# YimingQiao/Chunk-Compaction-in-Vectorized-Execution-SIMD

Measured on AMD Instinct MI355X. Metric: probe tuples/sec + achieved HBM GB/s, 1B-row int64 join at 1/2/4/8 GPUs, higher is better.
Workload: dtype int64; 1 GPU; C2: 1xMI355X linear-probe, 64M build / 1B probe int64 uniform keys, chunk=2048; table=linear_probing, layout=device, n_build=67108864, n_probe_per_gpu=1073741824, chunk=2048, parallelism=dp1

## Files before the change

chunk-compaction-in-vectorized-execution-simd_amd/ccj.py:

```python
from __future__ import annotations

import ctypes as C
import os
import subprocess

HERE = os.path.dirname(os.path.abspath(__file__))
LIB_PATH = os.environ.get("CCJ_LIB_PATH") or os.path.join(HERE, "libccj.so")

LP, CHAIN = 0, 1
LAYOUT_REFERENCE, LAYOUT_DEVICE = 0, 1
FLAG_CAP_OVERFLOW, FLAG_ROUND_OVERFLOW, FLAG_BAD_INPUT, FLAG_PART_OVERFLOW = 1, 2, 4, 8
PART_EXACT = 1
PART_ROWS = 2
PART_RANK = 4
PART_SHARE = 8

_lib = None
ABI_VERSION = 15


class CCJError(RuntimeError):
    pass


class TableInfo(C.Structure):
    _fields_ = [("kind", C.c_int32), ("layout", C.c_int32), ("n_keys", C.c_uint64), ("size", C.c_uint64),
                ("max_dup", C.c_uint64), ("max_rounds", C.c_uint32), ("reserved", C.c_uint32),
                ("d_table", C.c_void_p), ("d_bucket_off", C.c_void_p)]


class TableArrays(C.Structure):
    _fields_ = [("d_table", C.c_void_p), ("positions", C.c_uint64), ("d_row", C.c_void_p),
                ("d_bucket_off", C.c_void_p), ("d_bucket16", C.c_void_p), ("d_bucket8", C.c_void_p),
                ("n_bucket8", C.c_uint64), ("d_bucket_filter", C.c_void_p), ("n_filter_words", C.c_uint64)]


class ProbeArgs(C.Structure):
    _fields_ = [("keys", C.c_void_p), ("sel", C.c_void_p), ("counts", C.c_void_p), ("n_rows", C.c_uint64),
                ("chunk", C.c_uint32), ("max_rounds", C.c_uint32), ("cap", C.c_uint64),
                ("out_count", C.c_void_p), ("out_sel", C.c_void_p), ("out_payload", C.c_void_p),
                ("out_rounds", C.c_void_p), ("out_round_counts", C.c_void_p), ("status", C.c_void_p),
                ("out_pos", C.c_void_p), ("n_payload_cols", C.c_uint32), ("reserved2", C.c_uint32),
                ("out_payload_cols", C.c_void_p * 8)]


class CompactArgs(C.Structure):
    _fields_ = [("count", C.c_void_p), ("sel", C.c_void_p), ("payload", C.c_void_p), ("rounds", C.c_void_p),
                ("round_counts", C.c_void_p), ("n_chunks", C.c_uint64), ("cap", C.c_uint64),
                ("max_rounds", C.c_uint32), ("chunk", C.c_uint32), ("n_cols", C.c_uint32), ("threshold", C.c_uint32),
                ("cols", C.c_void_p * 16), ("out_cols", C.c_void_p * 16), ("out_payload", C.c_void_p),
                ("out_row", C.c_void_p), ("out_chunk_counts", C.c_void_p), ("out_cap_rows", C.c_uint64),
                ("out_n_chunks", C.c_void_p), ("workspace", C.c_void_p), ("workspace_bytes", C.c_size_t),
                ("status", C.c_void_p), ("key_cols", C.c_uint32)]


EXPORTS = ["ccj_last_error", "ccj_abi_version", "ccj_device_init", "ccj_table_build_reference",
           "ccj_table_build_from_host", "ccj_table_build_on_device", "ccj_table_get_info", "ccj_table_free",
           "ccj_probe", "ccj_gen_uniform_keys", "ccj_probe_cost", "ccj_result_checksum",
           "ccj_compact_workspace_size", "ccj_compact", "ccj_partition_workspace_size", "ccj_partition_by_owner",
           "ccj_result_checksum_mapped", "ccj_gen_reference_keys", "ccj_table_set_payload",
           "ccj_table_build_rank_index",
           "ccj_probe_partitioned_workspace_size", "ccj_probe_partitioned", "ccj_probe_partitioned_positions",
           "ccj_pipeline_create",
           "ccj_pipeline_run", "ccj_pipeline_free", "ccj_pipeline_checksum", "ccj_partition_by_owner_fixed",
           "ccj_segment_chunk_counts", "ccj_pipeline_set_thresholds", "ccj_gen_c3_keys",
           "ccj_partition_grouped_workspace_size", "ccj_partition_by_owner_grouped", "ccj_partition_grouped_sub_cap",
           "ccj_probe_ordered_workspace_size", "ccj_probe_ordered", "ccj_probe_visits",
           "ccj_stream_create_cu_masked", "ccj_stream_destroy", "ccj_device_cus", "ccj_copy_device",
           "ccj_table_get_arrays", "ccj_probe_cost_walk", "ccj_set_phase_events", "ccj_build_hash",
           "ccj_last_gather_kernel"]

MAX_JOINS = 8
COMPACT_NONE, COMPACT_FULL = 0, 1


class PipelineResult(C.Structure):
    _fields_ = [("n_out", C.c_uint64), ("cols", C.c_void_p * MAX_JOINS), ("payload", C.c_void_p * MAX_JOINS),
                ("chunks_in", C.c_uint64 * MAX_JOINS), ("rows_in", C.c_uint64 * MAX_JOINS),
                ("rows_out", C.c_uint64 * MAX_JOINS), ("level_ms", C.c_float * MAX_JOINS)]


def build(force: bool = False) -> str:
    if force or not os.path.exists(LIB_PATH):
        subprocess.run(["make", "-C", HERE, "-j8"], check=True)
    return LIB_PATH


def lib():
    global _lib
    if _lib is None:
        if not os.path.exists(LIB_PATH):
            raise CCJError(f"{LIB_PATH} missing: run `make -C {HERE}` (or __graft_entry__.build())")
        L = C.CDLL(LIB_PATH)
        vp, u64, i32 = C.c_void_p, C.c_uint64, C.c_int
        L.ccj_last_error.restype = C.c_char_p
        L.ccj_abi_version.restype = i32
        if L.ccj_abi_version() != ABI_VERSION:
            raise CCJError(f"{LIB_PATH} has ABI {L.ccj_abi_version()}, this binding needs {ABI_VERSION}: "
                           f"rebuild it (`make -C {HERE}`)")
        L.ccj_build_hash.restype = C.c_char_p
        L.ccj_last_gather_kernel.restype = C.c_char_p
        L.ccj_device_init.argtypes = [i32]
        L.ccj_table_build_reference.argtypes = [i32, u64, u64, i32, vp, C.POINTER(vp)]
        L.ccj_table_build_from_host.argtypes = [i32, vp, u64, C.POINTER(vp)]
        L.ccj_table_build_on_device.argtypes = [i32, vp, u64, vp, C.POINTER(vp)]
        L.ccj_table_get_info.argtypes = [vp, C.POINTER(TableInfo)]
        L.ccj_table_get_arrays.argtypes = [vp, C.POINTER(TableArrays)]
        L.ccj_table_free.argtypes = [vp]
        L.ccj_table_set_payload.argtypes = [vp, vp, C.c_uint32, vp]
        L.ccj_table_build_rank_index.argtypes = [vp, vp]
        L.ccj_probe_partitioned_workspace_size.restype = C.c_size_t
        L.ccj_probe_partitioned_workspace_size.argtypes = [vp, u64, C.c_uint32]
        L.ccj_probe_partitioned_positions.restype = u64
        L.ccj_probe_partitioned_positions.argtypes = [vp, u64, C.c_uint32]
        L.ccj_probe_partitioned.argtypes = [vp, C.POINTER(ProbeArgs), C.c_uint32, vp, vp, C.c_size_t, vp]
        L.ccj_probe.argtypes = [vp, C.POINTER(ProbeArgs), vp]
        L.ccj_probe_ordered_workspace_size.restype = C.c_size_t
        L.ccj_probe_ordered_workspace_size.argtypes = [vp, u64, C.c_uint32]
        L.ccj_probe_ordered.argtypes = [vp, C.POINTER(ProbeArgs), vp, C.c_size_t, vp]
        L.ccj_gen_uniform_keys.argtypes = [vp, u64, u64, u64, u64, vp]
        L.ccj_gen_reference_keys.argtypes = [vp, u64, u64, u64, u64, vp]
        L.ccj_gen_c3_keys.argtypes = [vp, u64, u64, u64, u64, u64, C.c_uint32, vp]
        L.ccj_probe_cost.argtypes = [vp, vp, u64, vp, vp]
        L.ccj_probe_cost_walk.argtypes = [vp, vp, u64, vp, vp]
        L.ccj_set_phase_events.argtypes = [C.POINTER(vp), C.c_uint32]
        L.ccj_probe_visits.argtypes = [vp, vp, vp, C.c_uint32, C.c_uint32, vp, vp, vp]
        L.ccj_compact_workspace_size.restype = C.c_size_t
        L.ccj_compact_workspace_size.argtypes = [u64, u64, C.c_uint32, C.c_uint32, C.c_uint32]
        L.ccj_compact.argtypes = [C.POINTER(CompactArgs), vp]
        L.ccj_partition_workspace_size.restype = C.c_size_t
        L.ccj_partition_workspace_size.argtypes = [u64, C.c_uint32]
# ... 135 lines not shown
        out = torch.empty(n, dtype=torch.int64, device=torch.device("cuda", torch.cuda.current_device()))
    check(lib().ccj_gen_c3_keys(_ptr(out), n, seed, first_row, n_build, cf, hit_ppm, _stream(stream)),
          "ccj_gen_c3_keys")
    return out


def gen_reference_keys(first: int, n: int, n_total: int, cf: int = 1, out=None, stream=None):
    import torch
    if out is None:
        out = torch.empty(n, dtype=torch.int64, device=torch.device("cuda", torch.cuda.current_device()))
    check(lib().ccj_gen_reference_keys(_ptr(out), first, n, n_total, cf, _stream(stream)), "ccj_gen_reference_keys")
    return out


class Table:
    def __init__(self, handle: C.c_void_p):
        self._h = handle
        info = TableInfo()
        check(lib().ccj_table_get_info(handle, C.byref(info)), "ccj_table_get_info")
        self.kind, self.layout = info.kind, info.layout
        self.n_keys, self.size = info.n_keys, info.size
        self.max_dup, self.max_rounds = info.max_dup, info.max_rounds
        self.d_table, self.d_bucket_off = info.d_table, info.d_bucket_off

    @classmethod
    def reference(cls, kind: int, n: int, cf: int = 1, layout: int = LAYOUT_REFERENCE, stream=None):
        h = C.c_void_p()
        check(lib().ccj_table_build_reference(kind, n, cf, layout, _stream(stream), C.byref(h)),
              "ccj_table_build_reference")
        return cls(h)

    @classmethod
    def from_host(cls, kind: int, keys):
        import numpy as np
        keys = np.ascontiguousarray(keys, dtype=np.int64)
        h = C.c_void_p()
        check(lib().ccj_table_build_from_host(kind, keys.ctypes.data_as(C.c_void_p), len(keys), C.byref(h)),
              "ccj_table_build_from_host")
        return cls(h)

    @classmethod
    def on_device(cls, kind: int, d_keys, stream=None):
        h = C.c_void_p()
        check(lib().ccj_table_build_on_device(kind, _ptr(d_keys), d_keys.numel(), _stream(stream), C.byref(h)),
              "ccj_table_build_on_device")
        return cls(h)

    def free(self):
        if self._h:
            lib().ccj_table_free(self._h)
            self._h = None

    def __del__(self):
        try:
            self.free()
        except Exception:
            pass

    def arrays(self):
        import numpy as np
        import torch
        a = TableArrays()
        check(lib().ccj_table_get_arrays(self._h, C.byref(a)), "ccj_table_get_arrays")
        torch.cuda.synchronize()

        def get(ptr, n, dt):
            return _d2h_bytes(ptr, n * np.dtype(dt).itemsize).view(dt)

        out = dict(table=get(a.d_table, a.positions, np.int64), row=get(a.d_row, a.positions, np.uint32))
# ... 414 lines not shown
```

chunk-compaction-in-vectorized-execution-simd_amd/csrc/ccj_api.hip:

```cpp
#include <algorithm>
#include <cstdlib>
#include <cstdio>
#include <cstring>
#include <map>
#include <memory>
#include <mutex>
#include <new>
#include <string>
#include <unordered_map>
#include <vector>

#include "ccj_internal.h"
#include "ccj_tuning.h"

namespace {

thread_local std::string g_err;

thread_local hipEvent_t g_phase[4] = {};
thread_local uint32_t g_n_phase = 0;
thread_local uint32_t g_phase_next = 0;
void phase_mark(hipStream_t s, uint32_t i) {
  if (i < g_n_phase && g_phase[i]) (void)hipEventRecord(g_phase[i], s);
  if (i + 1 > g_phase_next) g_phase_next = i + 1;
// ... 130 lines not shown
  if (e == hipSuccess) e = hipMalloc((void **)&t->d_ckeys, nck * 8);
  if (e == hipSuccess) e = ccj::launch_fill(t->d_ckeys, nck, -1, s);
  if (e == hipSuccess) e = ccj::launch_rank_index(t->d_table, size, t->d_occ, t->d_pre, cnt, s);
  if (e == hipSuccess) e = ccj::launch_rank_compact_keys(t->d_table, size, t->d_occ, t->d_pre, t->d_ckeys, s);
  if (e == hipSuccess) e = hipStreamSynchronize(s);
  if (cnt) (void)hipFree(cnt);
  if (e != hipSuccess) {
    for (void *q : {(void *)t->d_occ, (void *)t->d_pre, (void *)t->d_ckeys})
      if (q) (void)hipFree(q);
    t->d_occ = nullptr;
    t->d_pre = nullptr;
    t->d_ckeys = nullptr;
    return hip_fail(e, "LP window index");
  }
  t->rank_wbits = pl.window_bits;
  return CCJ_OK;
}
#else
int build_rank_index(ccj_table *, hipStream_t) {
  return fail(CCJ_ERR_INVALID, "ccj_table_build_rank_index: the rank walk is built into libccj_tuning.so only");
}
#endif

int build_lp_host(const int64_t *keys, uint64_t n, ccj_table **out) {
  const uint64_t size = lp_num_slots(n);
  if (size > (1ull << 32)) return fail(CCJ_ERR_LIMIT, "LP table larger than 2^32 slots");
  std::vector<int64_t> slots(size, -1);
  std::vector<uint32_t> rows(size < 4 ? 4 : size, ccj::kNoRow);
  const uint64_t mask = size - 1;
  for (uint64_t i = 0; i < n; ++i) {
    uint64_t s = ccj::murmurhash64((uint64_t)keys[i]) & mask;
    while (slots[s] != -1) s = (s + 1) & mask;
    slots[s] = keys[i];
    if (keys[i] != -1) rows[s] = (uint32_t)i;
  }
  std::unique_ptr<ccj_table> t(new ccj_table());
  t->info.kind = CCJ_TABLE_LP;
  t->info.layout = CCJ_LAYOUT_REFERENCE;
  t->info.n_keys = n;
  t->info.size = size;
  lp_host_stats(slots, &t->info.max_rounds, &t->info.max_dup);
  if (slots.size() < 4) slots.resize(4, -1);
  void *d = nullptr;
  int rc = upload(&d, slots.data(), slots.size() * sizeof(int64_t), "LP slots");
  if (rc) return rc;
  t->d_table = (int64_t *)d;
  t->positions = slots.size();
  rc = upload(&d, rows.data(), rows.size() * sizeof(uint32_t), "LP slot rows");
  if (rc) {
    (void)hipFree(t->d_table);
    return rc;
  }
  t->d_row = (uint32_t *)d;
  t->info.d_table = t->d_table;
  (void)hipGetDevice(&t->device);
  *out = t.release();
  return CCJ_OK;
}

int build_chain_host(const int64_t *keys, uint64_t n, ccj_table **out) {
  if (n >= (1ull << 32)) return fail(CCJ_ERR_LIMIT, "chaining table needs < 2^32 keys (uint32 CSR)");
  const uint64_t size = chain_num_buckets(n);
  const uint64_t mask = size - 1;
  std::vector<uint32_t> off(size + 1, 0);
  std::vector<uint32_t> bucket(n);
  for (uint64_t i = 0; i < n; ++i) {
    bucket[i] = (uint32_t)(ccj::murmurhash64((uint64_t)keys[i]) & mask);
    off[bucket[i] + 1]++;
  }
  uint32_t longest = 0;
  for (uint64_t b = 0; b < size; ++b) {
    longest = std::max(longest, off[b + 1]);
    off[b + 1] += off[b];
  }
  std::vector<int64_t> chain(n);
  std::vector<uint32_t> rows;
  {
    std::vector<uint32_t> fill(off.begin(), off.end() - 1);
// ... 134 lines not shown
  if (n_seg) best = std::max<uint64_t>(best, carry + st[0]);
  t->info.kind = CCJ_TABLE_LP;
  t->info.layout = CCJ_LAYOUT_DEVICE;
  t->info.n_keys = n;
  t->info.size = size;
  t->info.max_rounds = (uint32_t)best;
  uint64_t dup = known_dup;
  if (!dup && n) {
    uint32_t *d_dup = nullptr, h_dup = 0;
    e = hipMalloc(&d_dup, sizeof(uint32_t));
    if (e == hipSuccess) e = ccj::launch_lp_max_dup(t->d_table, size, (uint32_t)std::min<uint64_t>(best, size), d_dup, s);
    if (e == hipSuccess) e = hipMemcpyAsync(&h_dup, d_dup, sizeof(uint32_t), hipMemcpyDeviceToHost, s);
    if (e == hipSuccess) e = hipStreamSynchronize(s);
    if (d_dup) (void)hipFree(d_dup);
    if (e != hipSuccess) {
      cleanup();
      return hip_fail(e, "device LP build (max dup)");
    }
    dup = h_dup;
  }
  t->info.max_dup = dup ? dup : 1;
  t->info.d_table = t->d_table;
  (void)hipGetDevice(&t->device);
  *out = t.release();
  return CCJ_OK;
}

void zipf_table(uint64_t n, uint32_t *t) {
  double hn = 0.0;
  for (uint64_t r = 1; r <= n; ++r) hn += 1.0 / (double)r;
  uint32_t j = 0;
  double h = 0.0;
  for (uint64_t r = 1; r <= n && j < ccj::kZipfBuckets; ++r) {
    h += 1.0 / (double)r;
    while (j < ccj::kZipfBuckets && h * (double)ccj::kZipfBuckets > (double)j * hn) t[j++] = (uint32_t)r;
  }
  while (j < ccj::kZipfBuckets) t[j++] = (uint32_t)(n ? n : 1);
  t[ccj::kZipfBuckets] = (uint32_t)(n + 1);
}

}

extern "C" {

const char *ccj_last_error(void) { return g_err.c_str(); }

// ... 94 lines not shown
    return fail(CCJ_ERR_INVALID, "ccj_table_set_payload: bad argument");
  if (!t->d_row) return fail(CCJ_ERR_INVALID, "ccj_table_set_payload: table has no row map");
  void *d = nullptr;
  if (hipMalloc(&d, t->positions * n_cols * sizeof(int64_t)) != hipSuccess)
    return fail(CCJ_ERR_OOM, "payload: hipMalloc failed");
  hipError_t e = ccj::launch_scatter_payload(d_payload, n_cols, t->d_row, t->positions, (int64_t *)d,
                                             (hipStream_t)stream);
  if (e == hipSuccess) e = hipStreamSynchronize((hipStream_t)stream);
  if (e != hipSuccess) {
    (void)hipFree(d);
    return hip_fail(e, "payload scatter");
  }
  if (t->d_pay) (void)hipFree(t->d_pay);
  t->d_pay = (int64_t *)d;
  t->n_pay = n_cols;
  return CCJ_OK;
}

int ccj_table_build_rank_index(ccj_table *t, ccj_stream stream) {
  if (!t) return fail(CCJ_ERR_INVALID, "ccj_table_build_rank_index: null table");
  return build_rank_index(t, (hipStream_t)stream);
}

int ccj_table_free(ccj_table *t) {
  if (!t) return CCJ_OK;
  if (t->d_table) (void)hipFree(t->d_table);
  if (t->d_off) (void)hipFree(t->d_off);
  if (t->d_bucket) (void)hipFree(t->d_bucket);
  if (t->d_bucket8) (void)hipFree(t->d_bucket8);
  if (t->d_filt) (void)hipFree(t->d_filt);
  if (t->d_row) (void)hipFree(t->d_row);
  if (t->d_pay) (void)hipFree(t->d_pay);
  if (t->d_occ) (void)hipFree(t->d_occ);
  if (t->d_pre) (void)hipFree(t->d_pre);
  if (t->d_ckeys) (void)hipFree(t->d_ckeys);
  delete t;
  return CCJ_OK;
}

namespace {
int fill_probe_params(const ccj_table *t, const ccj_probe_args *a, ccj::ProbeParams &p) {
  if (!t || !a) return fail(CCJ_ERR_INVALID, "ccj_probe: null table/args");
  if (a->chunk == 0 || a->chunk > ccj::kMaxChunk) return fail(CCJ_ERR_INVALID, "ccj_probe: chunk must be 1..2048");
  if (a->out_round_counts && a->max_rounds == 0) return fail(CCJ_ERR_INVALID, "ccj_probe: max_rounds == 0");
  if (a->n_rows && (!a->out_count || !a->out_sel || !a->keys))
    return fail(CCJ_ERR_INVALID, "ccj_probe: missing buffer");
  p = ccj::ProbeParams{};
  p.table = t->d_table;
// ... 79 lines not shown
  const size_t rank = 0;
  (void)t;
#endif
  return align256(L.positions * 8) + align256(fixed > exact ? fixed : exact) + rank;
}
size_t part_ws_sub_bytes(const ccj_table *t, const PartLayout &L, uint32_t chunk) {
  if (!t->n_pay || !L.pl.lo_bits) return 0;
  const uint64_t out_chunks = (L.positions + chunk - 1) / chunk;
  return align256(out_chunks * 8 * 4);
}
}

size_t ccj_probe_partitioned_workspace_size(const ccj_table *t, uint64_t n_rows, uint32_t chunk) {
  if (!t) return 0;
  const PartLayout L = part_layout(t, n_rows, chunk);
  return part_ws_base_bytes(t, L, n_rows) + part_ws_sub_bytes(t, L, chunk);
}

int ccj_probe_partitioned(const ccj_table *t, const ccj_probe_args *a, uint32_t flags, uint32_t *out_row_map,
                          void *ws, size_t ws_bytes, ccj_stream stream) {
  PhaseScope phase_scope((hipStream_t)stream);
  ccj::ProbeParams p;
  if (int rc = fill_probe_params(t, a, p)) return rc;
  if (t->info.kind == CCJ_TABLE_CHAIN && (a->out_pos || a->n_payload_cols))
    return fail(CCJ_ERR_INVALID, "ccj_probe_partitioned: positions / payload columns need an LP table");
  if (a->sel) return fail(CCJ_ERR_INVALID, "ccj_probe_partitioned: sel must be NULL");
  if (a->counts && (flags & CCJ_PART_EXACT))
    return fail(CCJ_ERR_INVALID, "ccj_probe_partitioned: input chunk counts need the one-pass split (no CCJ_PART_EXACT)");
  if (a->out_round_counts)
    return fail(CCJ_ERR_INVALID, "ccj_probe_partitioned: no round counts (no Next boundaries in partition order)");
  if ((a->out_pos || a->n_payload_cols) && t->info.size < 16)
    return fail(CCJ_ERR_INVALID, "ccj_probe_partitioned: positions / payload columns need a table of >= 16 slots");
  if (a->n_rows >= (1ull << 32)) return fail(CCJ_ERR_LIMIT, "ccj_probe_partitioned: n_rows must be < 2^32");
  if (flags & ~(CCJ_PART_EXACT | CCJ_PART_ROWS | CCJ_PART_RANK | CCJ_PART_SHARE))
    return fail(CCJ_ERR_INVALID, "ccj_probe_partitioned: unknown flags");
#ifdef CCJ_RANK_WALK
  if ((flags & CCJ_PART_RANK) && !t->d_ckeys && rank_index_applies(t))
    return fail(CCJ_ERR_INVALID, "ccj_probe_partitioned: CCJ_PART_RANK needs ccj_table_build_rank_index first");
#else
  if (flags & CCJ_PART_RANK)
    return fail(CCJ_ERR_INVALID, "ccj_probe_partitioned: CCJ_PART_RANK: the rank walk is built into libccj_tuning.so only");
#endif
  const bool rows = (flags & CCJ_PART_ROWS) != 0;
  if (rows && (!a->out_payload || p.cap != a->chunk || t->info.max_dup > 1 || t->info.kind != CCJ_TABLE_LP ||
               t->info.size < 16 || ((a->out_pos || a->n_payload_cols) && t->info.size > (1ull << 31))))
    return fail(CCJ_ERR_INVALID, "ccj_probe_partitioned: CCJ_PART_ROWS needs an LP table of >= 16 slots with distinct "
// ... 516 lines not shown
```

chunk-compaction-in-vectorized-execution-simd_amd/csrc/ccj_internal.h:

```cpp
#pragma once

#include <hip/hip_runtime.h>

#include <cstdint>
#include <string>

#include "ccj.h"

struct ccj_table {
  ccj_table_info info;
  int64_t *d_table = nullptr;
  uint32_t *d_off = nullptr;
  int64_t *d_bucket = nullptr;
  uint64_t *d_bucket8 = nullptr;
  uint32_t *d_filt = nullptr;
  uint32_t *d_row = nullptr;
  uint64_t positions = 0;
  int64_t *d_pay = nullptr;
  uint32_t n_pay = 0;
  int device = 0;
  uint64_t *d_occ = nullptr;
  uint32_t *d_pre = nullptr;
  int64_t *d_ckeys = nullptr;
  uint32_t rank_wbits = 0;
};

namespace ccj {

__host__ __device__ __forceinline__ uint64_t murmurhash64(uint64_t x) {
  x ^= x >> 32;
  x *= 0xd6e8feb86659fd93ULL;
  x ^= x >> 32;
  x *= 0xd6e8feb86659fd93ULL;
  x ^= x >> 32;
  return x;
}

__host__ __device__ __forceinline__ uint32_t murmurhash64_hi(uint64_t x) {
  constexpr uint64_t kC = 0xd6e8feb86659fd93ULL;
  x ^= x >> 32;
  x *= kC;
  x ^= x >> 32;
  const uint32_t lo = (uint32_t)x, hi = (uint32_t)(x >> 32);
  return (uint32_t)(((uint64_t)lo * (uint32_t)kC) >> 32) + lo * (uint32_t)(kC >> 32) + hi * (uint32_t)kC;
}

__host__ __device__ __forceinline__ uint32_t bucket_fp(uint64_t h) { return (uint32_t)(h >> 52); }
__host__ __device__ __forceinline__ uint32_t rec8_first(uint64_t r, uint32_t kfp) {
  const uint32_t st = (uint32_t)r, len = (uint32_t)(r >> 32) & 0xFFu;
  const bool m0 = ((uint32_t)(r >> 40) & 0xFFFu) == kfp;
  const bool m1 = len >= 2u && ((uint32_t)(r >> 52) & 0xFFFu) == kfp;
  const uint32_t c = m0 ? st : m1 ? st + 1u : st + 2u;
  return c < st + len ? c : st + len;
}

constexpr int kWave = 64;
constexpr int kWavesPerBlock = 4;
constexpr uint32_t kMaxChunk = 2048;
constexpr uint32_t kMaxParts = 64;

struct ProbeParams {
  const int64_t *table;
  const uint32_t *off;
  const longlong2 *bucket;
  const uint64_t *bucket8;
  uint32_t mask;
  const int64_t *keys;
  const uint32_t *sel;
  const uint32_t *counts;
  uint64_t n_rows;
  uint64_t n_chunks;
  uint32_t chunk;
  uint32_t max_rounds;
  uint64_t cap;
  uint32_t *out_count;
  uint32_t *out_sel;
  int64_t *out_payload;
  uint32_t *out_rounds;
  uint32_t *out_round_counts;
  uint32_t *status;
  uint32_t *out_pos;
  const int64_t *pay;
  uint32_t n_pay;
  uint32_t pay_stride;
  int64_t *out_cols[CCJ_MAX_PAYLOAD_COLS];
// ... 30 lines not shown

hipError_t launch_probe(int kind, const ProbeParams &p, hipStream_t s);
hipError_t launch_probe_flat(int kind, const ProbeParams &p, hipStream_t s);
hipError_t launch_ordered_walk(int kind, const ProbeParams &p, hipStream_t s);
uint32_t stream_cus(hipStream_t s);
hipError_t launch_unsplit_words(const uint2 *runs, const uint32_t *ovf_runs, const uint16_t *row_loc,
                                const void *w_pos, void *w_row, uint64_t n, uint32_t parts, uint32_t tile,
                                uint32_t *status, hipStream_t s, bool w16);
hipError_t launch_ordered_emit(int kind, const ProbeParams &p, hipStream_t s);
hipError_t launch_gather_payload(const ProbeParams &p, const uint32_t *pos, hipStream_t s, uint32_t parts = 0,
                                 uint64_t cpp = 0);
const char *last_gather_kernel();
hipError_t launch_gen_reference_keys(int64_t *out, uint64_t first, uint64_t n, uint64_t n_total, uint64_t cf,
                                     hipStream_t s);
hipError_t launch_fill(int64_t *p, uint64_t n, int64_t v, hipStream_t s);
hipError_t launch_iota_u32(uint32_t *p, uint64_t n, hipStream_t s);
hipError_t launch_copy16(const void *src, void *dst, uint64_t n16, hipStream_t s);
hipError_t launch_lp_insert(const int64_t *keys, uint64_t n, int64_t *slots, uint32_t *slot_row, uint32_t mask,
                            hipStream_t s);
hipError_t launch_scatter_payload(const int64_t *src, uint32_t n_cols, const uint32_t *row, uint64_t positions,
                                  int64_t *dst, hipStream_t s);
hipError_t launch_lp_max_dup(const int64_t *slots, uint64_t n_slots, uint32_t max_run, uint32_t *out, hipStream_t s);
hipError_t launch_lp_runs(const int64_t *slots, uint64_t n_slots, uint32_t *seg_stats, hipStream_t s);
int build_chain_device(const int64_t *d_keys, uint64_t n, hipStream_t s, uint64_t known_dup, ccj_table **out);
hipError_t build_chain_filter(ccj_table *t, hipStream_t s);
constexpr uint64_t kRunSegment = 4096;
hipError_t launch_gen_c3(int64_t *out, uint64_t n, uint64_t seed, uint64_t first_row, uint64_t n_build, uint64_t cf,
                         uint32_t hit_ppm, const uint32_t *zipf, hipStream_t s);
constexpr uint32_t kZipfBits = 16, kZipfBuckets = 1u << kZipfBits;
hipError_t launch_gen_uniform(int64_t *out, uint64_t n, uint64_t seed, uint64_t first_row, uint64_t range,
                              hipStream_t s);
hipError_t launch_probe_visits(int kind, const int64_t *table, const uint32_t *off, uint32_t mask,
                               const int64_t *keys, const uint32_t *sel, uint32_t count, uint32_t max_rounds,
                               int64_t *vals, uint32_t *len, hipStream_t s);
hipError_t launch_probe_cost(int kind, const int64_t *table, const uint32_t *off, uint32_t mask,
                             const int64_t *keys, uint64_t n, unsigned long long *acc, hipStream_t s,
                             bool walk = false);
hipError_t launch_result_checksum(const uint32_t *count, const uint32_t *sel, const int64_t *payload,
                                  uint64_t n_chunks, uint64_t cap, uint32_t chunk, uint64_t row_base,
                                  const uint64_t *row_map, unsigned long long *acc, hipStream_t s);

int api_fail(int code, const std::string &msg);
int api_check_device();

size_t compact_workspace(uint64_t n_chunks, uint64_t cap, uint32_t chunk, uint32_t max_rounds, uint32_t threshold);
hipError_t launch_compact(const ccj_compact_args &a, hipStream_t s);
// ... 72 lines not shown
```

chunk-compaction-in-vectorized-execution-simd_amd/csrc/ccj_kernels.hip:

```cpp
#include <cstdlib>
#include <string>

#include "ccj_internal.h"
#include "ccj_tuning.h"

namespace ccj {
namespace {

__device__ __forceinline__ uint32_t lane_prefix(uint64_t m) {
  return __builtin_amdgcn_mbcnt_hi((uint32_t)(m >> 32), __builtin_amdgcn_mbcnt_lo((uint32_t)m, 0u));
}

template <int KIND>
__device__ __forceinline__ void emit_extra(const ProbeParams &p, uint64_t obase, uint64_t o, int64_t k, uint32_t r) {
  if (!p.out_pos && p.n_pay == 0) return;
  const uint32_t h = (uint32_t)murmurhash64((uint64_t)k) & p.mask;
  const uint32_t pos = KIND == CCJ_TABLE_LP ? ((h + r) & p.mask) : p.off[h] + r;
  if (p.out_pos) p.out_pos[obase + o] = pos;
  if (p.n_pay) {
    const int64_t *row = p.pay + (uint64_t)pos * p.pay_stride;
    for (uint32_t c = 0; c < p.n_pay; ++c) p.out_cols[c][obase + o] = row[c];
  }
}

// ... 2428 lines not shown
      walk_finish(p, sm, c, lane, lane_rounds, 0u, t0, t1, t2, steps);
      return;
    }
  }
  const uint32_t overflow = walk_emit<kWaveRows>(p, sm, c, w0, wend, lane);
  walk_finish(p, sm, c, lane, lane_rounds, overflow, t0, t1, t2, steps);
}

#ifdef CCJ_TUNING
template <int AUX, int KJ>
__device__ __forceinline__ void stage_keys_aux(const int64_t *keys, uint32_t phys, uint32_t w0, uint32_t wend,
                                               uint32_t lane, int64_t (&k)[KJ]) {
  const auto rs = __builtin_amdgcn_make_buffer_rsrc(const_cast<int64_t *>(keys), (short)0, (int)(phys * 8), 0x00020000);
#pragma unroll
  for (int j = 0; j < KJ; ++j) {
    const uint32_t i = w0 + (uint32_t)(j >> 1) * 128u + 2u * lane + (uint32_t)(j & 1);
    k[j] = (int64_t)__builtin_amdgcn_raw_buffer_load_b64(rs, (int)(i * 8), 0, AUX);
  }
#pragma unroll
  for (int j = 0; j < KJ; ++j)
    if (w0 + (uint32_t)(j >> 1) * 128u + 2u * lane + (uint32_t)(j & 1) >= wend) k[j] = 0;
}
#endif
template <bool POS, int NB = 1>
__global__ __launch_bounds__(kWave * 4, POS && NB == 1 ? 5 : 1) void probe_walk2(ProbeParams p) {
  constexpr int NW = 4;
  constexpr uint32_t kWaveRows = kMaxChunk / NW;
  constexpr int kJ = (int)(kWaveRows / kWave);
  __shared__ Walk1Shared<NB, NW> sm;
  const uint32_t tid = threadIdx.x, lane = tid & (kWave - 1), wave = tid / kWave;
  unsigned long long t0, t1, t2;
  uint32_t steps = 0;
  CCJ_STAMP(t0);
  const uint64_t c = walk_chunk_index(p);
  const uint64_t base = c * p.chunk;
  const uint32_t phys = flat_phys(p, base);
  const uint32_t w0 = wave * kWaveRows;
  const uint32_t wend = phys > w0 ? (phys - w0 < kWaveRows ? phys : w0 + kWaveRows) : w0;
  auto row_of = [&](int j) { return w0 + (uint32_t)(j >> 1) * 128u + 2u * lane + (uint32_t)(j & 1); };
  int64_t k[kJ];
  uint32_t h[kJ];
#ifdef CCJ_TUNING
  if (p.key_aux == 0u) {
#endif
    typedef long long i64x2 __attribute__((ext_vector_type(2)));
    const bool a16 = ((uintptr_t)(p.keys + base) & 15u) == 0u;
#pragma unroll
    for (int j = 0; j < kJ; j += 2) {
      const uint32_t i = row_of(j);
// ... 7 lines not shown
      case 1: stage_keys_aux<1>(p.keys + base, phys, w0, wend, lane, k); break;
      case 2: stage_keys_aux<2>(p.keys + base, phys, w0, wend, lane, k); break;
      case 3: stage_keys_aux<3>(p.keys + base, phys, w0, wend, lane, k); break;
      case 16: stage_keys_aux<16>(p.keys + base, phys, w0, wend, lane, k); break;
      case 17: stage_keys_aux<17>(p.keys + base, phys, w0, wend, lane, k); break;
      case 18: stage_keys_aux<18>(p.keys + base, phys, w0, wend, lane, k); break;
      case 19: stage_keys_aux<19>(p.keys + base, phys, w0, wend, lane, k); break;
      default: stage_keys_aux<0>(p.keys + base, phys, w0, wend, lane, k); break;
    }
  }
#endif
#pragma unroll
  for (int j = 0; j < kJ; ++j) {
    sm.key[row_of(j)] = k[j];
    h[j] = (uint32_t)murmurhash64((uint64_t)k[j]) & p.mask;
  }
  uint32_t rid_e[kJ];
  if (POS && p.out_sub) load_emit_rows(p, c, w0, wend, lane, rid_e);
  CCJ_STAMP(t1);
  char *ring = sm.ring + wave * NB * kRingSlot;
  const uint32_t ring_lds = (uint32_t)__builtin_amdgcn_readfirstlane(
      (int)(uint32_t)(uintptr_t)(__attribute__((address_space(3))) char *)ring);
  const char *win = ring + (lane & 1u) * 1024 + (lane >> 1) * 32;
  const uint32_t last_start = p.mask - (kWin - 1);
  const uint32_t half = (lane & 1u) * 2u;
  auto start = [&](uint32_t cur) {
    uint32_t s = cur < last_start ? cur : last_start;
    const uint32_t lim = (s & ~15u) + (16u - kWin);
    return s < lim ? s : lim;
  };
  auto issue = [&](uint32_t a, uint32_t slot) {
    uint32_t a0 = (uint32_t)__builtin_amdgcn_mov_dpp((int)a, 0xA0, 0xF, 0xF, false);
    uint32_t a1 = (uint32_t)__builtin_amdgcn_mov_dpp((int)a, 0xF5, 0xF, 0xF, false);
    dpp_check(p, a, a0, a1, lane);
    a0 = a0 < last_start ? a0 : last_start;
    a1 = a1 < last_start ? a1 : last_start;
    dma16(p.table + a0 + half, ring_lds + slot * kRingSlot);
    dma16(p.table + a1 + half, ring_lds + slot * kRingSlot + 1024u);
  };
  auto look = [&](int64_t kk, uint32_t cur, uint32_t s, uint32_t &hits, uint32_t slot) {
    const longlong2 x0 = *reinterpret_cast<const longlong2 *>(win + slot * kRingSlot);
    const longlong2 x1 = *reinterpret_cast<const longlong2 *>(win + slot * kRingSlot + 16);
    const uint32_t e = (x0.x == -1 ? 1u : 0u) | (x0.y == -1 ? 2u : 0u) | (x1.x == -1 ? 4u : 0u) | (x1.y == -1 ? 8u : 0u);
    const uint32_t m = (x0.x == kk ? 1u : 0u) | (x0.y == kk ? 2u : 0u) | (x1.x == kk ? 4u : 0u) | (x1.y == kk ? 8u : 0u);
    const uint32_t off = cur - s;
    const uint32_t ee = e >> off;
    const uint32_t f = (uint32_t)__builtin_ctz(ee | ((1u << kWin) >> off));
    hits = (m >> off) & ((1u << f) - 1u);
    return ee != 0u || hits != 0u;
  };
  auto result = [&](uint32_t cur, uint32_t hits) {
    return POS ? (hits ? (cur + (uint32_t)__builtin_ctz(hits)) | 0x80000000u : 0u) : (hits ? 1u : 0u);
  };

  uint32_t cont = 0;
  uint32_t sa[kJ];
#pragma unroll
  for (int j = 0; j < kJ; ++j) sa[j] = start(h[j]);
  if (NB > 1) issue(w0 < wend ? sa[0] : 0u, 0u);
#pragma unroll
  for (int j = 0; j < kJ; ++j) {
    ++steps;
    const uint32_t i = row_of(j);
    const bool valid = i < wend;
    const uint32_t s = sa[j];
    if (NB > 1) {
      if (j + 1 < kJ) {
        issue(row_of(j + 1) < wend ? sa[j + 1] : 0u, (uint32_t)(j + 1) & 1u);
        wait_vmcnt<2>();
      } else {
        wait_vmcnt<0>();
      }
    } else {
      issue(valid ? s : 0u, 0u);
      wait_vmcnt<0>();
    }
    if (valid) {
      uint32_t hits;
      if (look(k[j], h[j], s, hits, NB > 1 ? (uint32_t)j & 1u : 0u)) {
        sm.hc[i] = result(h[j], hits);
      } else {
        sm.hc[i] = (s + kWin) & p.mask;
        cont |= 1u << j;
      }
    }
  }
  if (__ballot(cont != 0u)) {
    bool have = false;
    uint32_t bi = 0, bcur = 0, bst = 0;
    int64_t bkey = 0;
    auto take = [&]() {
      if (!have && cont) {
        const int j = __builtin_ctz(cont);
        cont &= cont - 1u;
        bi = row_of(j);
        bkey = sm.key[bi];
        bcur = sm.hc[bi];
        have = true;
      }
    };
    take();
    bst = start(bcur);
    issue(have ? bst : 0u, 0u);
    for (bool more = true; more;) {
      ++steps;
      wait_vmcnt<0>();
      if (have) {
        uint32_t hits;
        if (look(bkey, bcur, bst, hits, 0u)) {
          sm.hc[bi] = result(bcur, hits);
          have = false;
        } else {
          bcur = (bst + kWin) & p.mask;
        }
      }
      take();
      if (__ballot(have) == 0ull) {
        more = false;
        break;
      }
      bst = start(bcur);
      issue(have ? bst : 0u, 0u);
    }
  }
  CCJ_STAMP(t2);
  __syncthreads();
  if (tid == 0) {
    sm.total = 0;
    sm.rounds = 0;
  }
  __syncthreads();
  if (POS) {
    if (p.out_sub) walk_emit_pos_sub<kWaveRows, NW>(p, sm, c, w0, wend, lane, wave, rid_e);
    else walk_emit_pos<kWaveRows, NW>(p, sm, c, w0, wend, lane, wave, sm.wtot, phys);
    walk_finish(p, sm, c, lane, 0u, 0u, t0, t1, t2, steps);
    return;
// ... 259 lines not shown
hipError_t launch_probe_flat(int kind, const ProbeParams &p, hipStream_t s) {
  if (p.n_chunks == 0) return hipSuccess;
  const dim3 g((unsigned)p.n_chunks), b(kFlatThreads);
  const uint64_t size = (uint64_t)p.mask + 1;
  if (kind != CCJ_TABLE_LP) {
    if (!p.bucket) return hipErrorInvalidValue;
    if (chain_filt_applies(p, kFiltUnit) && !p.out_rounds && ccj_tune_int("CCJ_CHAIN_FILT", 1)) {
      hipError_t e = hipMemsetAsync(p.out_count, 0, p.n_chunks * sizeof(uint32_t), s);
      if (e != hipSuccess) return e;
      const uint32_t grid = std::max<uint32_t>(8u, 2 * stream_cus(s) / 8 * 8);
      hipLaunchKernelGGL(probe_chain_filt, dim3(grid), dim3(kFiltThreads), 0, s, p);
      ProbeParams q = p;
      q.chunk0 = p.ovf_base / p.chunk;
      q.xcd_swizzle = 0;
      if (p.n_chunks > q.chunk0)
        hipLaunchKernelGGL((probe_chain_win<3>), dim3((unsigned)(p.n_chunks - q.chunk0)), b, 0, s, q);
      return hipGetLastError();
    }
    hipLaunchKernelGGL((probe_chain_win<3>), g, b, 0, s, p);
    return hipGetLastError();
  }
  if (size < 16) return launch_probe(kind, p, s);
  const bool walk2 = p.first_match && ccj_tune_int("CCJ_WALK2", 1);
  if (p.out_pos && p.rows_in_sel) {
    if (walk2 && ccj_tune_int("CCJ_WALK2_POS_NB", 1) == 2) hipLaunchKernelGGL((probe_walk2<true, 2>), g, b, 0, s, p);
    else if (walk2) hipLaunchKernelGGL((probe_walk2<true>), g, b, 0, s, p);
    else hipLaunchKernelGGL((probe_walk1<1, false, true>), g, b, 0, s, p);
  } else if (p.out_pos) {
    hipLaunchKernelGGL((probe_win<3>), g, b, 0, s, p);
  } else {
    if (ccj_tune_int("CCJ_WALK_LANES", 2) == 4)
      hipLaunchKernelGGL((probe_walk<3, true, 4, false, 4>), g, b, 0, s, p);
    else if (ccj_tune_int("CCJ_WALK_DMA", 2) == 0)
      hipLaunchKernelGGL((probe_walk<3, true>), g, b, 0, s, p);
    else if (ccj_tune_int("CCJ_WALK_DMA", 2) == 1)
      hipLaunchKernelGGL((probe_walk<3, true, 4, false, 2, true>), g, b, 0, s, p);
    else if (ccj_tune_int("CCJ_WALK_NB", 1) == 2)
      hipLaunchKernelGGL((probe_walk1<2>), g, b, 0, s, p);
    else if (ccj_tune_int("CCJ_WALK_NB", 1) == 3)
      hipLaunchKernelGGL((probe_walk1<3>), g, b, 0, s, p);
    else if (walk2 && ccj_tune_int("CCJ_WALK2_NB", 2) == 1)
      hipLaunchKernelGGL((probe_walk2<false, 1>), g, b, 0, s, p);
    else if (walk2)
      hipLaunchKernelGGL((probe_walk2<false, 2>), g, b, 0, s, p);
    else if (ccj_tune_int("CCJ_WALK_NW", 4) == 8)
      hipLaunchKernelGGL((probe_walk1<1, false, false, 8>), g, dim3(kWave * 8), 0, s, p);
    else
      hipLaunchKernelGGL((probe_walk1<1>), g, b, 0, s, p);
  }
  return hipGetLastError();
}

namespace {
struct GatherParams {
  const uint32_t *count, *pos;
  const uint64_t *out_base;
  uint64_t cap;
  const int64_t *pay;
  uint32_t stride;
  int64_t *cols[CCJ_MAX_PAYLOAD_COLS];
  uint32_t shift;
  uint32_t mask;
  uint32_t ablate;
  const uint32_t *sub;
  uint32_t parts, groups;
// ... 507 lines not shown
      const int64_t v = slots[(i + t) & mask];
      if (v == -1) break;
      c += v == k;
    }
    best = c > best ? c : best;
  }
  for (int d = 32; d > 0; d >>= 1) {
    const uint32_t o = (uint32_t)__shfl_xor((int)best, d);
    best = o > best ? o : best;
  }
  if ((threadIdx.x & 63u) == 0 && best) atomicMax(out, best);
}
}

hipError_t launch_lp_max_dup(const int64_t *slots, uint64_t n_slots, uint32_t max_run, uint32_t *out, hipStream_t s) {
  hipError_t e = hipMemsetAsync(out, 0, sizeof(uint32_t), s);
  if (e != hipSuccess || n_slots == 0) return e;
  const uint64_t want = (n_slots + 255) / 256;
  hipLaunchKernelGGL(lp_max_dup, dim3((unsigned)(want < 8192 ? want : 8192)), dim3(256), 0, s, slots, n_slots,
                     max_run, out);
  return hipGetLastError();
}

hipError_t launch_lp_runs(const int64_t *slots, uint64_t n_slots, uint32_t *seg_stats, hipStream_t s) {
  const uint64_t n_seg = (n_slots + kRunSegment - 1) / kRunSegment;
  hipLaunchKernelGGL(lp_runs, dim3((unsigned)((n_seg + 3) / 4)), dim3(256), 0, s, slots, n_slots, seg_stats);
  return hipGetLastError();
}

}
```

include/ccj.h:

```cpp
#ifndef CCJ_H
#define CCJ_H

#include <stddef.h>
#include <stdint.h>

#ifdef __cplusplus
extern "C" {
#endif

#define CCJ_ABI_VERSION 15

enum ccj_status {
  CCJ_OK = 0,
  CCJ_ERR_INVALID = -1,
  CCJ_ERR_HIP = -2,
  CCJ_ERR_NO_DEVICE = -3,
  CCJ_ERR_OOM = -4,
  CCJ_ERR_LIMIT = -5
};

enum ccj_flag {
  CCJ_FLAG_CAP_OVERFLOW = 1u,
  CCJ_FLAG_ROUND_OVERFLOW = 2u,
  CCJ_FLAG_BAD_INPUT = 4u,
// ... 2 lines not shown
};

enum ccj_table_kind {
  CCJ_TABLE_LP = 0,
  CCJ_TABLE_CHAIN = 1
};

enum ccj_layout {
  CCJ_LAYOUT_REFERENCE = 0,
  CCJ_LAYOUT_DEVICE = 1
};

typedef void *ccj_stream;
#define CCJ_MAX_PAYLOAD_COLS 8
typedef struct ccj_table ccj_table;

typedef struct ccj_table_info {
  int32_t kind;
  int32_t layout;
  uint64_t n_keys;
  uint64_t size;
  uint64_t max_dup;
  uint32_t max_rounds;
  uint32_t reserved;
  const int64_t *d_table;
  const uint32_t *d_bucket_off;
} ccj_table_info;

const char *ccj_last_error(void);
int ccj_abi_version(void);
const char *ccj_build_hash(void);
const char *ccj_last_gather_kernel(void);
int ccj_set_phase_events(void *const *events, uint32_t n);
int ccj_device_init(int device);

int ccj_table_build_reference(int kind, uint64_t n_rhs_tuples, uint64_t chunk_factor, int layout,
                              ccj_stream stream, ccj_table **out);
int ccj_table_build_from_host(int kind, const int64_t *h_keys, uint64_t n, ccj_table **out);
int ccj_table_build_on_device(int kind, const int64_t *d_keys, uint64_t n, ccj_stream stream,
                              ccj_table **out);
int ccj_table_get_info(const ccj_table *table, ccj_table_info *info);
typedef struct ccj_table_arrays {
  const int64_t *d_table;
  uint64_t positions;
  const uint32_t *d_row;
  const uint32_t *d_bucket_off;
  const int64_t *d_bucket16;
  const uint64_t *d_bucket8;
  uint64_t n_bucket8;
  const uint32_t *d_bucket_filter;
  uint64_t n_filter_words;
} ccj_table_arrays;
int ccj_table_get_arrays(const ccj_table *table, ccj_table_arrays *arrays);
int ccj_table_set_payload(ccj_table *table, const int64_t *d_payload, uint32_t n_cols, ccj_stream stream);
int ccj_table_free(ccj_table *table);
int ccj_table_build_rank_index(ccj_table *table, ccj_stream stream);

typedef struct ccj_probe_args {
  const int64_t *keys;
  const uint32_t *sel;
  const uint32_t *counts;
  uint64_t n_rows;
  uint32_t chunk;
  uint32_t max_rounds;
  uint64_t cap;
  uint32_t *out_count;
  uint32_t *out_sel;
  int64_t *out_payload;
  uint32_t *out_rounds;
  uint32_t *out_round_counts;
  uint32_t *status;
  uint32_t *out_pos;
  uint32_t n_payload_cols;
  uint32_t reserved2;
  int64_t *out_payload_cols[CCJ_MAX_PAYLOAD_COLS];
} ccj_probe_args;

int ccj_probe(const ccj_table *table, const ccj_probe_args *args, ccj_stream stream);
// ... 112 lines not shown
```

Baseline: 98.02 billion probe tuples/s.

## Add compact 32-bit slot array for linear-probe table and probe it

When every build key fits in 32 bits and the table is unique-key linear probing, the build step now creates a parallel uint32 copy of the slot array, with all-ones marking empty slots. The walk2 probe kernel can read this copy instead of the int64 table. Each 32-byte DMA window then covers 8 slots instead of 4, which halves the table bytes touched per probe and the table's cache footprint. Probe keys outside 32-bit range are treated as misses. The cost is extra device memory and a conversion pass at build time, and the new path is only wired through the partitioned probe entry point.

```diff
diff --git a/chunk-compaction-in-vectorized-execution-simd_amd/ccj.py b/chunk-compaction-in-vectorized-execution-simd_amd/ccj.py
--- a/chunk-compaction-in-vectorized-execution-simd_amd/ccj.py
+++ b/chunk-compaction-in-vectorized-execution-simd_amd/ccj.py
@@ -25,7 +25,7 @@
 
 class TableInfo(C.Structure):
     _fields_ = [("kind", C.c_int32), ("layout", C.c_int32), ("n_keys", C.c_uint64), ("size", C.c_uint64),
-                ("max_dup", C.c_uint64), ("max_rounds", C.c_uint32), ("reserved", C.c_uint32),
+                ("max_dup", C.c_uint64), ("max_rounds", C.c_uint32), ("slot32", C.c_uint32),
                 ("d_table", C.c_void_p), ("d_bucket_off", C.c_void_p)]
 
 
@@ -68,7 +68,7 @@
            "ccj_probe_ordered_workspace_size", "ccj_probe_ordered", "ccj_probe_visits",
            "ccj_stream_create_cu_masked", "ccj_stream_destroy", "ccj_device_cus", "ccj_copy_device",
            "ccj_table_get_arrays", "ccj_probe_cost_walk", "ccj_set_phase_events", "ccj_build_hash",
-           "ccj_last_gather_kernel"]
+           "ccj_last_gather_kernel", "ccj_table_drop_slot32"]
 
 MAX_JOINS = 8
 COMPACT_NONE, COMPACT_FULL = 0, 1
@@ -107,6 +107,8 @@
         L.ccj_table_get_info.argtypes = [vp, C.POINTER(TableInfo)]
         L.ccj_table_get_arrays.argtypes = [vp, C.POINTER(TableArrays)]
         L.ccj_table_free.argtypes = [vp]
+        if hasattr(L, "ccj_table_drop_slot32"):
+            L.ccj_table_drop_slot32.argtypes = [vp]
         L.ccj_table_set_payload.argtypes = [vp, vp, C.c_uint32, vp]
         L.ccj_table_build_rank_index.argtypes = [vp, vp]
         L.ccj_probe_partitioned_workspace_size.restype = C.c_size_t
@@ -288,6 +290,7 @@
         self.n_keys, self.size = info.n_keys, info.size
         self.max_dup, self.max_rounds = info.max_dup, info.max_rounds
         self.d_table, self.d_bucket_off = info.d_table, info.d_bucket_off
+        self.slot32 = bool(info.slot32)
 
     @classmethod
     def reference(cls, kind: int, n: int, cf: int = 1, layout: int = LAYOUT_REFERENCE, stream=None):
@@ -311,6 +314,10 @@
         check(lib().ccj_table_build_on_device(kind, _ptr(d_keys), d_keys.numel(), _stream(stream), C.byref(h)),
               "ccj_table_build_on_device")
         return cls(h)
+
+    def drop_slot32(self):
+        check(lib().ccj_table_drop_slot32(self._h), "ccj_table_drop_slot32")
+        self.slot32 = False
 
     def free(self):
         if self._h:
diff --git a/chunk-compaction-in-vectorized-execution-simd_amd/csrc/ccj_api.hip b/chunk-compaction-in-vectorized-execution-simd_amd/csrc/ccj_api.hip
--- a/chunk-compaction-in-vectorized-execution-simd_amd/csrc/ccj_api.hip
+++ b/chunk-compaction-in-vectorized-execution-simd_amd/csrc/ccj_api.hip
@@ -176,6 +176,29 @@
 }
 #endif
 
+int build_slot32(ccj_table *t, hipStream_t s) {
+  t->info.slot32 = 0;
+  if (t->info.kind != CCJ_TABLE_LP || t->info.max_dup > 1 || t->info.size < 32 || t->d_slot32) return CCJ_OK;
+  const uint64_t size = t->info.size;
+  uint32_t *d32 = nullptr, *d_bad = nullptr, h_bad = 1;
+  if (hipMalloc((void **)&d32, size * sizeof(uint32_t)) != hipSuccess) {
+    (void)hipGetLastError();
+    return CCJ_OK;
+  }
+  hipError_t e = hipMalloc((void **)&d_bad, sizeof(uint32_t));
+  if (e == hipSuccess) e = ccj::launch_lp_slot32(t->d_table, size, d32, d_bad, s);
+  if (e == hipSuccess) e = hipMemcpyAsync(&h_bad, d_bad, sizeof(uint32_t), hipMemcpyDeviceToHost, s);
+  if (e == hipSuccess) e = hipStreamSynchronize(s);
+  if (d_bad) (void)hipFree(d_bad);
+  if (e != hipSuccess || h_bad) {
+    (void)hipFree(d32);
+    return e != hipSuccess ? hip_fail(e, "LP 32-bit slot array") : CCJ_OK;
+  }
+  t->d_slot32 = d32;
+  t->info.slot32 = 1;
+  return CCJ_OK;
+}
+
 int build_lp_host(const int64_t *keys, uint64_t n, ccj_table **out) {
   const uint64_t size = lp_num_slots(n);
   if (size > (1ull << 32)) return fail(CCJ_ERR_LIMIT, "LP table larger than 2^32 slots");
@@ -208,6 +231,12 @@
   t->d_row = (uint32_t *)d;
   t->info.d_table = t->d_table;
   (void)hipGetDevice(&t->device);
+  rc = build_slot32(t.get(), nullptr);
+  if (rc) {
+    (void)hipFree(t->d_table);
+    (void)hipFree(t->d_row);
+    return rc;
+  }
   *out = t.release();
   return CCJ_OK;
 }
@@ -388,6 +417,10 @@
   t->info.max_dup = dup ? dup : 1;
   t->info.d_table = t->d_table;
   (void)hipGetDevice(&t->device);
+  if (int rc = build_slot32(t.get(), s)) {
+    cleanup();
+    return rc;
+  }
   *out = t.release();
   return CCJ_OK;
 }
@@ -528,8 +561,17 @@
   return build_rank_index(t, (hipStream_t)stream);
 }
 
+int ccj_table_drop_slot32(ccj_table *t) {
+  if (!t) return CCJ_OK;
+  if (t->d_slot32) (void)hipFree(t->d_slot32);
+  t->d_slot32 = nullptr;
+  t->info.slot32 = 0;
+  return CCJ_OK;
+}
+
 int ccj_table_free(ccj_table *t) {
   if (!t) return CCJ_OK;
+  if (t->d_slot32) (void)hipFree(t->d_slot32);
   if (t->d_table) (void)hipFree(t->d_table);
   if (t->d_off) (void)hipFree(t->d_off);
   if (t->d_bucket) (void)hipFree(t->d_bucket);
@@ -655,6 +697,7 @@
   PhaseScope phase_scope((hipStream_t)stream);
   ccj::ProbeParams p;
   if (int rc = fill_probe_params(t, a, p)) return rc;
+  p.table32 = t->d_slot32;
   if (t->info.kind == CCJ_TABLE_CHAIN && (a->out_pos || a->n_payload_cols))
     return fail(CCJ_ERR_INVALID, "ccj_probe_partitioned: positions / payload columns need an LP table");
   if (a->sel) return fail(CCJ_ERR_INVALID, "ccj_probe_partitioned: sel must be NULL");
diff --git a/chunk-compaction-in-vectorized-execution-simd_amd/csrc/ccj_internal.h b/chunk-compaction-in-vectorized-execution-simd_amd/csrc/ccj_internal.h
--- a/chunk-compaction-in-vectorized-execution-simd_amd/csrc/ccj_internal.h
+++ b/chunk-compaction-in-vectorized-execution-simd_amd/csrc/ccj_internal.h
@@ -23,6 +23,7 @@
   uint32_t *d_pre = nullptr;
   int64_t *d_ckeys = nullptr;
   uint32_t rank_wbits = 0;
+  uint32_t *d_slot32 = nullptr;
 };
 
 namespace ccj {
@@ -61,6 +62,7 @@
 
 struct ProbeParams {
   const int64_t *table;
+  const uint32_t *table32;
   const uint32_t *off;
   const longlong2 *bucket;
   const uint64_t *bucket8;
@@ -137,6 +139,7 @@
                                   int64_t *dst, hipStream_t s);
 hipError_t launch_lp_max_dup(const int64_t *slots, uint64_t n_slots, uint32_t max_run, uint32_t *out, hipStream_t s);
 hipError_t launch_lp_runs(const int64_t *slots, uint64_t n_slots, uint32_t *seg_stats, hipStream_t s);
+hipError_t launch_lp_slot32(const int64_t *slots, uint64_t n_slots, uint32_t *slot32, uint32_t *bad, hipStream_t s);
 int build_chain_device(const int64_t *d_keys, uint64_t n, hipStream_t s, uint64_t known_dup, ccj_table **out);
 hipError_t build_chain_filter(ccj_table *t, hipStream_t s);
 constexpr uint64_t kRunSegment = 4096;
diff --git a/chunk-compaction-in-vectorized-execution-simd_amd/csrc/ccj_kernels.hip b/chunk-compaction-in-vectorized-execution-simd_amd/csrc/ccj_kernels.hip
--- a/chunk-compaction-in-vectorized-execution-simd_amd/csrc/ccj_kernels.hip
+++ b/chunk-compaction-in-vectorized-execution-simd_amd/csrc/ccj_kernels.hip
@@ -2474,9 +2474,11 @@
     if (w0 + (uint32_t)(j >> 1) * 128u + 2u * lane + (uint32_t)(j & 1) >= wend) k[j] = 0;
 }
 #endif
-template <bool POS, int NB = 1>
+template <bool POS, int NB = 1, bool S32 = false>
 __global__ __launch_bounds__(kWave * 4, POS && NB == 1 ? 5 : 1) void probe_walk2(ProbeParams p) {
   constexpr int NW = 4;
+  constexpr uint32_t kW = S32 ? 8u : (uint32_t)kWin;
+  constexpr uint32_t kLine = S32 ? 32u : 16u;
   constexpr uint32_t kWaveRows = kMaxChunk / NW;
   constexpr int kJ = (int)(kWaveRows / kWave);
   __shared__ Walk1Shared<NB, NW> sm;
@@ -2530,30 +2532,47 @@
   const uint32_t ring_lds = (uint32_t)__builtin_amdgcn_readfirstlane(
       (int)(uint32_t)(uintptr_t)(__attribute__((address_space(3))) char *)ring);
   const char *win = ring + (lane & 1u) * 1024 + (lane >> 1) * 32;
-  const uint32_t last_start = p.mask - (kWin - 1);
-  const uint32_t half = (lane & 1u) * 2u;
+  const uint32_t last_start = p.mask - (kW - 1u);
+  const uint32_t half = (lane & 1u) * (kW / 2u);
   auto start = [&](uint32_t cur) {
     uint32_t s = cur < last_start ? cur : last_start;
-    const uint32_t lim = (s & ~15u) + (16u - kWin);
+    const uint32_t lim = (s & ~(kLine - 1u)) + (kLine - kW);
     return s < lim ? s : lim;
   };
+  auto in_range = [&](int64_t kk) { return !S32 || ((uint64_t)kk >> 32) == 0u; };
   auto issue = [&](uint32_t a, uint32_t slot) {
     uint32_t a0 = (uint32_t)__builtin_amdgcn_mov_dpp((int)a, 0xA0, 0xF, 0xF, false);
     uint32_t a1 = (uint32_t)__builtin_amdgcn_mov_dpp((int)a, 0xF5, 0xF, 0xF, false);
     dpp_check(p, a, a0, a1, lane);
     a0 = a0 < last_start ? a0 : last_start;
     a1 = a1 < last_start ? a1 : last_start;
-    dma16(p.table + a0 + half, ring_lds + slot * kRingSlot);
-    dma16(p.table + a1 + half, ring_lds + slot * kRingSlot + 1024u);
+    if (S32) {
+      dma16(p.table32 + a0 + half, ring_lds + slot * kRingSlot);
+      dma16(p.table32 + a1 + half, ring_lds + slot * kRingSlot + 1024u);
+    } else {
+      dma16(p.table + a0 + half, ring_lds + slot * kRingSlot);
+      dma16(p.table + a1 + half, ring_lds + slot * kRingSlot + 1024u);
+    }
   };
   auto look = [&](int64_t kk, uint32_t cur, uint32_t s, uint32_t &hits, uint32_t slot) {
-    const longlong2 x0 = *reinterpret_cast<const longlong2 *>(win + slot * kRingSlot);
-    const longlong2 x1 = *reinterpret_cast<const longlong2 *>(win + slot * kRingSlot + 16);
-    const uint32_t e = (x0.x == -1 ? 1u : 0u) | (x0.y == -1 ? 2u : 0u) | (x1.x == -1 ? 4u : 0u) | (x1.y == -1 ? 8u : 0u);
-    const uint32_t m = (x0.x == kk ? 1u : 0u) | (x0.y == kk ? 2u : 0u) | (x1.x == kk ? 4u : 0u) | (x1.y == kk ? 8u : 0u);
+    uint32_t e, m;
+    if (S32) {
+      const uint4 y0 = *reinterpret_cast<const uint4 *>(win + slot * kRingSlot);
+      const uint4 y1 = *reinterpret_cast<const uint4 *>(win + slot * kRingSlot + 16);
+      const uint32_t k32 = (uint32_t)kk, none = 0xFFFFFFFFu;
+      e = (y0.x == none ? 1u : 0u) | (y0.y == none ? 2u : 0u) | (y0.z == none ? 4u : 0u) | (y0.w == none ? 8u : 0u) |
+          (y1.x == none ? 16u : 0u) | (y1.y == none ? 32u : 0u) | (y1.z == none ? 64u : 0u) | (y1.w == none ? 128u : 0u);
+      m = (y0.x == k32 ? 1u : 0u) | (y0.y == k32 ? 2u : 0u) | (y0.z == k32 ? 4u : 0u) | (y0.w == k32 ? 8u : 0u) |
+          (y1.x == k32 ? 16u : 0u) | (y1.y == k32 ? 32u : 0u) | (y1.z == k32 ? 64u : 0u) | (y1.w == k32 ? 128u : 0u);
+    } else {
+      const longlong2 x0 = *reinterpret_cast<const longlong2 *>(win + slot * kRingSlot);
+      const longlong2 x1 = *reinterpret_cast<const longlong2 *>(win + slot * kRingSlot + 16);
+      e = (x0.x == -1 ? 1u : 0u) | (x0.y == -1 ? 2u : 0u) | (x1.x == -1 ? 4u : 0u) | (x1.y == -1 ? 8u : 0u);
+      m = (x0.x == kk ? 1u : 0u) | (x0.y == kk ? 2u : 0u) | (x1.x == kk ? 4u : 0u) | (x1.y == kk ? 8u : 0u);
+    }
     const uint32_t off = cur - s;
     const uint32_t ee = e >> off;
-    const uint32_t f = (uint32_t)__builtin_ctz(ee | ((1u << kWin) >> off));
+    const uint32_t f = (uint32_t)__builtin_ctz(ee | ((1u << kW) >> off));
     hits = (m >> off) & ((1u << f) - 1u);
     return ee != 0u || hits != 0u;
   };
@@ -2564,7 +2583,7 @@
   uint32_t cont = 0;
   uint32_t sa[kJ];
 #pragma unroll
-  for (int j = 0; j < kJ; ++j) sa[j] = start(h[j]);
+  for (int j = 0; j < kJ; ++j) sa[j] = in_range(k[j]) ? start(h[j]) : 0u;
   if (NB > 1) issue(w0 < wend ? sa[0] : 0u, 0u);
 #pragma unroll
   for (int j = 0; j < kJ; ++j) {
@@ -2585,10 +2604,12 @@
     }
     if (valid) {
       uint32_t hits;
-      if (look(k[j], h[j], s, hits, NB > 1 ? (uint32_t)j & 1u : 0u)) {
+      if (!in_range(k[j])) {
+        sm.hc[i] = result(h[j], 0u);
+      } else if (look(k[j], h[j], s, hits, NB > 1 ? (uint32_t)j & 1u : 0u)) {
         sm.hc[i] = result(h[j], hits);
       } else {
-        sm.hc[i] = (s + kWin) & p.mask;
+        sm.hc[i] = (s + kW) & p.mask;
         cont |= 1u << j;
       }
     }
@@ -2619,7 +2640,7 @@
           sm.hc[bi] = result(bcur, hits);
           have = false;
         } else {
-          bcur = (bst + kWin) & p.mask;
+          bcur = (bst + kW) & p.mask;
         }
       }
       take();
@@ -2925,8 +2946,12 @@
   }
   if (size < 16) return launch_probe(kind, p, s);
   const bool walk2 = p.first_match && ccj_tune_int("CCJ_WALK2", 1);
+  const bool s32 = walk2 && p.table32 && size >= 32 && ccj_tune_int("CCJ_SLOT32", 1);
   if (p.out_pos && p.rows_in_sel) {
-    if (walk2 && ccj_tune_int("CCJ_WALK2_POS_NB", 1) == 2) hipLaunchKernelGGL((probe_walk2<true, 2>), g, b, 0, s, p);
+    if (walk2 && ccj_tune_int("CCJ_WALK2_POS_NB", 1) == 2) {
+      if (s32) hipLaunchKernelGGL((probe_walk2<true, 2, true>), g, b, 0, s, p);
+      else hipLaunchKernelGGL((probe_walk2<true, 2>), g, b, 0, s, p);
+    } else if (walk2 && s32) hipLaunchKernelGGL((probe_walk2<true, 1, true>), g, b, 0, s, p);
     else if (walk2) hipLaunchKernelGGL((probe_walk2<true>), g, b, 0, s, p);
     else hipLaunchKernelGGL((probe_walk1<1, false, true>), g, b, 0, s, p);
   } else if (p.out_pos) {
@@ -2942,8 +2967,11 @@
       hipLaunchKernelGGL((probe_walk1<2>), g, b, 0, s, p);
     else if (ccj_tune_int("CCJ_WALK_NB", 1) == 3)
       hipLaunchKernelGGL((probe_walk1<3>), g, b, 0, s, p);
-    else if (walk2 && ccj_tune_int("CCJ_WALK2_NB", 2) == 1)
-      hipLaunchKernelGGL((probe_walk2<false, 1>), g, b, 0, s, p);
+    else if (walk2 && ccj_tune_int("CCJ_WALK2_NB", 2) == 1) {
+      if (s32) hipLaunchKernelGGL((probe_walk2<false, 1, true>), g, b, 0, s, p);
+      else hipLaunchKernelGGL((probe_walk2<false, 1>), g, b, 0, s, p);
+    } else if (walk2 && s32)
+      hipLaunchKernelGGL((probe_walk2<false, 2, true>), g, b, 0, s, p);
     else if (walk2)
       hipLaunchKernelGGL((probe_walk2<false, 2>), g, b, 0, s, p);
     else if (ccj_tune_int("CCJ_WALK_NW", 4) == 8)
@@ -3497,6 +3525,28 @@
   return hipGetLastError();
 }
 
+namespace {
+__global__ __launch_bounds__(256) void lp_slot32(const int64_t *slots, uint64_t n_slots, uint32_t *out, uint32_t *bad) {
+  bool b = false;
+  for (uint64_t i = (uint64_t)blockIdx.x * blockDim.x + threadIdx.x; i < n_slots;
+       i += (uint64_t)gridDim.x * blockDim.x) {
+    const int64_t k = slots[i];
+    b = b || (k != -1 && (uint64_t)k > 0xFFFFFFFEull);
+    out[i] = k == -1 ? 0xFFFFFFFFu : (uint32_t)k;
+  }
+  if (__ballot(b) != 0ull && (threadIdx.x & 63u) == 0u) atomicOr(bad, 1u);
+}
+}
+
+hipError_t launch_lp_slot32(const int64_t *slots, uint64_t n_slots, uint32_t *slot32, uint32_t *bad, hipStream_t s) {
+  hipError_t e = hipMemsetAsync(bad, 0, sizeof(uint32_t), s);
+  if (e != hipSuccess || n_slots == 0) return e;
+  const uint64_t want = (n_slots + 255) / 256;
+  hipLaunchKernelGGL(lp_slot32, dim3((unsigned)(want < 16384 ? want : 16384)), dim3(256), 0, s, slots, n_slots,
+                     slot32, bad);
+  return hipGetLastError();
+}
+
 hipError_t launch_lp_runs(const int64_t *slots, uint64_t n_slots, uint32_t *seg_stats, hipStream_t s) {
   const uint64_t n_seg = (n_slots + kRunSegment - 1) / kRunSegment;
   hipLaunchKernelGGL(lp_runs, dim3((unsigned)((n_seg + 3) / 4)), dim3(256), 0, s, slots, n_slots, seg_stats);
diff --git a/include/ccj.h b/include/ccj.h
--- a/include/ccj.h
+++ b/include/ccj.h
@@ -48,7 +48,7 @@
   uint64_t size;
   uint64_t max_dup;
   uint32_t max_rounds;
-  uint32_t reserved;
+  uint32_t slot32;
   const int64_t *d_table;
   const uint32_t *d_bucket_off;
 } ccj_table_info;
@@ -80,6 +80,7 @@
 int ccj_table_get_arrays(const ccj_table *table, ccj_table_arrays *arrays);
 int ccj_table_set_payload(ccj_table *table, const int64_t *d_payload, uint32_t n_cols, ccj_stream stream);
 int ccj_table_free(ccj_table *table);
+int ccj_table_drop_slot32(ccj_table *table);
 int ccj_table_build_rank_index(ccj_table *table, ccj_stream stream);
 
 typedef struct ccj_probe_args {
```

New measurement: 103.3 billion probe tuples/s (median of 6 runs). +5.4%, better.
